# stella-cv/stella_vslam

Measured on AMD Instinct MI355X. Metric: frames/s ORB-extract+match @640x480,2k kpts, higher is better.
Workload: dtype u8

## Files before the change

stella_vslam_amd/csrc/orb_kernels.hip:

```cpp
#include "svgpu_internal.h"
#include "sv_trig.h"
#include <utility>

#pragma clang fp contract(off)

namespace {

__device__ __constant__ float c_pattern_f[1024] = {
#include "orb_pattern_i8.inc"
};

__device__ __forceinline__ int find_level(const OrbLevel* __restrict__ L, int num_levels, int idx, int OrbLevel::*first,
                                          int* local) {
    int lv = 0;
    for (int l = 0; l < num_levels; ++l) {
        const int f = L[l].*first;
        if (idx >= f) lv = l;
    }
    *local = idx - L[lv].*first;
    return lv;
}

__device__ __forceinline__ int reflect101(int p, int len) {
    if (len == 1) return 0;
// ... 261 lines not shown
    }
    else if (MODE == BLUR_EDGE) {
        if (e.left) {
            const uint32_t* p = reinterpret_cast<const uint32_t*>(row);
            r.w1 = p[0];
            r.w2 = p[1];
            r.w0 = __builtin_amdgcn_perm(r.w2, r.w1, 0x01020304u);
        }
        else {
            const uint32_t* p = reinterpret_cast<const uint32_t*>(row + x0 - 4);
            const uint32_t pm1 = p[0], p0 = p[1], p1 = e.hi_p1 ? p[2] : 0u;
            r.w0 = pm1;
            r.w1 = __builtin_amdgcn_perm(p0, pm1, e.sel1);
            r.w2 = e.hi_p1 ? __builtin_amdgcn_perm(p1, p0, e.sel2) : __builtin_amdgcn_perm(p0, pm1, e.sel2);
        }
    }
    else {
        uint32_t b[12];
#pragma unroll
        for (int k = 0; k < 12; ++k) b[k] = row[reflect101(x0 - 4 + k, w)];
        r.w0 = b[0] | (b[1] << 8) | (b[2] << 16) | (b[3] << 24);
        r.w1 = b[4] | (b[5] << 8) | (b[6] << 16) | (b[7] << 24);
        r.w2 = b[8] | (b[9] << 8) | (b[10] << 16) | (b[11] << 24);
    }
    return r;
}
constexpr uint32_t BLUR_TAPS[7] = {18, 34, 48, 56, 48, 34, 18};
constexpr uint32_t blur_tap_word(int j, int word) {
    uint32_t t = 0;
    for (int k = 0; k < 4; ++k) {
        const int i = 4 * word + k - j - 1;
        if (i >= 0 && i < 7) t |= BLUR_TAPS[i] << (8 * k);
    }
    return t;
}
static_assert(blur_tap_word(0, 0) == 0x30221200u && blur_tap_word(0, 1) == 0x12223038u && blur_tap_word(0, 2) == 0u && blur_tap_word(3, 0) == 0u &&
              blur_tap_word(3, 1) == 0x38302212u && blur_tap_word(3, 2) == 0x00122230u, "blur tap words");
template <int J>
__device__ __forceinline__ uint32_t blur_hsum(const BlurRow& r) {
    constexpr uint32_t t0 = blur_tap_word(J, 0), t1 = blur_tap_word(J, 1), t2 = blur_tap_word(J, 2);
    uint32_t s = __builtin_amdgcn_udot4(r.w1, t1, 0u, false);
    if (t0) s = __builtin_amdgcn_udot4(r.w0, t0, s, false);
    if (t2) s = __builtin_amdgcn_udot4(r.w2, t2, s, false);
    return s;
}
__device__ __forceinline__ void blur_hpair(const BlurRow& a, const BlurRow& b, u16x2 (&hp)[4]) {
    hp[0] = as_u16x2(blur_hsum<0>(a) | (blur_hsum<0>(b) << 16));
    hp[1] = as_u16x2(blur_hsum<1>(a) | (blur_hsum<1>(b) << 16));
    hp[2] = as_u16x2(blur_hsum<2>(a) | (blur_hsum<2>(b) << 16));
    hp[3] = as_u16x2(blur_hsum<3>(a) | (blur_hsum<3>(b) << 16));
}
__device__ __forceinline__ uint32_t blur_dot(u16x2 h, uint32_t taps, uint32_t acc) { return __builtin_amdgcn_udot2(h, as_u16x2(taps), acc, false); }
__device__ __forceinline__ uint32_t blur_pack(const uint32_t (&acc)[4]) {
    const uint32_t lo = __builtin_amdgcn_perm(acc[1], acc[0], 0x0c0c0602u), hi = __builtin_amdgcn_perm(acc[3], acc[2], 0x06020c0cu);
    return lo | hi;
}

template <int MODE, int PAIRS = 0, class LoadPair>
__device__ __forceinline__ void blur_walk(LoadPair load_pair, uint8_t* __restrict__ Dp, int dpitch, int ys, int ye) {
    constexpr int AHEAD = MODE == BLUR_LDS ? 0 : 2;
    u16x2 A[4], B[4], C[4], D[4], E[4];
    BlurRow n0 = {}, n1 = {};
    {
        BlurRow r[8];
#pragma unroll
        for (int k = 0; k < 4; ++k) load_pair(ys - 4 + 2 * k, r[2 * k], r[2 * k + 1]);
        if (AHEAD) load_pair(ys + 4, n0, n1);
        if (MODE == BLUR_INTERIOR) {
#pragma unroll
            for (int k = 0; k < 8; ++k) asm volatile("" : "+v"(r[k].w0), "+v"(r[k].w1), "+v"(r[k].w2));
            asm volatile("" : "+v"(n0.w0), "+v"(n0.w1), "+v"(n0.w2), "+v"(n1.w0), "+v"(n1.w1), "+v"(n1.w2));
        }
        blur_hpair(r[0], r[1], A);
        blur_hpair(r[2], r[3], B);
        blur_hpair(r[4], r[5], C);
        blur_hpair(r[6], r[7], D);
    }
    auto step = [&](int y, bool second) {
        const BlurRow c0 = n0, c1 = n1;
        load_pair(y + 4 + AHEAD, n0, n1);
        if (AHEAD) blur_hpair(c0, c1, E);
        else blur_hpair(n0, n1, E);
        uint32_t acc[4];
#pragma unroll
        for (int j = 0; j < 4; ++j)
            acc[j] = blur_dot(D[j], 34u | (18u << 16), blur_dot(C[j], 56u | (48u << 16), blur_dot(B[j], 34u | (48u << 16), blur_dot(A[j], 18u << 16, 32768u))));
        *reinterpret_cast<uint32_t*>(Dp + __umul24(y, dpitch)) = blur_pack(acc);
        if (second) {
#pragma unroll
            for (int j = 0; j < 4; ++j)
                acc[j] = blur_dot(E[j], 18u, blur_dot(D[j], 48u | (34u << 16), blur_dot(C[j], 48u | (56u << 16), blur_dot(B[j], 18u | (34u << 16), 32768u))));
            *reinterpret_cast<uint32_t*>(Dp + __umul24(y + 1, dpitch)) = blur_pack(acc);
        }
#pragma unroll
        for (int j = 0; j < 4; ++j) {
            A[j] = B[j];
            B[j] = C[j];
            C[j] = D[j];
            D[j] = E[j];
        }
    };
    if constexpr (PAIRS > 0) {
#pragma unroll
        for (int i = 0; i < PAIRS; ++i) step(ys + 2 * i, true);
    }
    else
        for (int y = ys; y < ye; y += 2) step(y, y + 1 < ye);
}
template <int MODE>
__device__ __forceinline__ void blur_strip(const uint8_t* __restrict__ src, int spitch, int w, int h, uint8_t* __restrict__ dst,
                                           int dpitch, int x0, int ys, int ye) {
    auto row_ptr = [&](int y) { return src + __umul24(reflect101(y, h), spitch); };
    BlurEdge edge = {};
    if (MODE == BLUR_EDGE) edge = blur_edge_ctx(x0, w);
    blur_walk<MODE>([&](int y, BlurRow& a, BlurRow& b) {
        a = blur_load<MODE>(row_ptr(y), x0, w, edge);
        b = blur_load<MODE>(row_ptr(y + 1), x0, w, edge);
    }, dst + x0, dpitch, ys, ye);
}

__device__ __forceinline__ void blur_locate(const OrbLevel* __restrict__ L, int num_levels, const uint8_t* __restrict__ img0,
                                            size_t img0_frame_stride, int img0_pitch, const uint8_t* __restrict__ pyr,
                                            size_t pyr_frame_bytes, uint8_t* __restrict__ blur, size_t blur_frame_bytes, OrbLevel& lev,
                                            int& tile, const uint8_t*& src, int& spitch, uint8_t*& dst,
                                            int OrbLevel::*first = &OrbLevel::btile_first) {
    int b, item;
    xcd_frame_map(gridDim.x, gridDim.y, item, b);
    const int lv = find_level(L, num_levels, item, first, &tile);
    lev = L[lv];
    if (lv == 0) {
        src = img0 + (size_t)b * img0_frame_stride;
        spitch = img0_pitch;
    }
    else {
        src = pyr + (size_t)b * pyr_frame_bytes + lev.pyr_off;
        spitch = lev.pitch;
    }
    dst = blur + (size_t)b * blur_frame_bytes + lev.blur_off;
}
__device__ __forceinline__ bool blur_streamable(const uint8_t* src, int spitch, int w) {
    return ((((size_t)src) | (size_t)spitch) & 3) == 0 && w >= 16;
}
template <int ROWS>
__global__ __launch_bounds__(256) void k_blur(const OrbLevel* __restrict__ L, int num_levels, const uint8_t* __restrict__ img0,
                                              size_t img0_frame_stride, int img0_pitch, const uint8_t* __restrict__ pyr,
                                              size_t pyr_frame_bytes, uint8_t* __restrict__ blur, size_t blur_frame_bytes) {
    OrbLevel lev;
    int tile, spitch;
    const uint8_t* src;
    uint8_t* dst;
    blur_locate(L, num_levels, img0, img0_frame_stride, img0_pitch, pyr, pyr_frame_bytes, blur, blur_frame_bytes, lev, tile, src, spitch, dst);
    if (!blur_streamable(src, spitch, lev.w)) return;
    const int main_tiles = lev.btiles_x * lev.btiles_y;
    if (tile < main_tiles) {
        const int tx = tile % lev.btiles_x, ty = tile / lev.btiles_x;
        const int rem_groups = tx == lev.btiles_x - 1 ? (min(lev.w - 6, (tx + 1) * BLUR_TW) - tx * BLUR_TW + 3) / 4 : 64;
        int g = 64;
        while (g > 1 && (g >> 1) >= rem_groups) g >>= 1;
        if (g <= 32 && rem_groups > 0) {
            const int spw = 64 / g, lane = threadIdx.x & 63;
            if (ty * spw >= lev.btiles_y) return;
            const int strip = (ty * 4 + (int)(threadIdx.x >> 6)) * spw + lane / g;
            const int x0 = tx * BLUR_TW + (lane % g) * 4, ys = strip * ROWS;
            if (x0 >= lev.w || ys >= lev.h) return;
            if (x0 >= 4 && x0 + 6 < lev.w) blur_strip<BLUR_INTERIOR>(src, spitch, lev.w, lev.h, dst, lev.pitch, x0, ys, min(ys + ROWS, lev.h));
            return;
        }
        const int x0 = tx * BLUR_TW + (threadIdx.x & 63) * 4;
        const int ys = __builtin_amdgcn_readfirstlane(ty * (4 * ROWS) + (int)(threadIdx.x >> 6) * ROWS);
        if (x0 >= lev.w || ys >= lev.h) return;
        if (x0 >= 4 && x0 + 6 < lev.w) blur_strip<BLUR_INTERIOR>(src, spitch, lev.w, lev.h, dst, lev.pitch, x0, ys, min(ys + ROWS, lev.h));
    }
    else {
        const int which = threadIdx.x & 3, strip = (tile - main_tiles) * 64 + (threadIdx.x >> 2);
        const int ys = strip * BLUR_EDGE_ROWS;
        const int last = ((lev.w - 1) >> 2) << 2;
        int x0;
        if (which == 0) x0 = 0;
        else if (which == 1) x0 = last;
        else if (which == 2) x0 = last - 4;
        else return;
        if (ys >= lev.h || x0 < 0 || (which != 0 && (x0 == 0 || x0 + 6 < lev.w))) return;
        blur_strip<BLUR_EDGE>(src, spitch, lev.w, lev.h, dst, lev.pitch, x0, ys, min(ys + BLUR_EDGE_ROWS, lev.h));
    }
}
#define BLUR_LP (16 + BLUR_SEG + 16)
#define BLUR_LDS_ROWS (BLUR_ROWS + 8)
static_assert(BLUR_SEG % 16 == 0 && BLUR_BAND_THREADS % 64 == 0 && BLUR_SEG / 4 <= BLUR_BAND_THREADS && BLUR_ROWS % 2 == 0, "blur band geometry");
static_assert(BLUR_LDS_ROWS * BLUR_LP <= 64 * 1024, "blur band exceeds the static LDS limit");
constexpr int blur_chunks(int groups, int rows) {
    const int fit = BLUR_BAND_THREADS / groups, pairs = rows >> 1, c = fit < pairs ? fit : pairs;
    return c > 1 ? c : 1;
}
constexpr int blur_chunk_rows(int groups, int rows) { return ((rows + blur_chunks(groups, rows) - 1) / blur_chunks(groups, rows) + 1) & ~1; }
constexpr int BLUR_FULL_RC = blur_chunk_rows(BLUR_SEG / 4, BLUR_ROWS);
template <>
__global__ __launch_bounds__(BLUR_BAND_THREADS) void k_blur<BLUR_ROWS>(const OrbLevel* __restrict__ L, int num_levels, const uint8_t* __restrict__ img0,
                                                                       size_t img0_frame_stride, int img0_pitch, const uint8_t* __restrict__ pyr,
                                                                       size_t pyr_frame_bytes, uint8_t* __restrict__ blur, size_t blur_frame_bytes) {
    __shared__ __attribute__((aligned(16))) uint8_t s_rows[BLUR_LDS_ROWS * BLUR_LP];
    OrbLevel lev;
    int item, spitch;
    const uint8_t* src;
    uint8_t* dst;
    blur_locate(L, num_levels, img0, img0_frame_stride, img0_pitch, pyr, pyr_frame_bytes, blur, blur_frame_bytes, lev, item, src, spitch, dst,
                &OrbLevel::bband_first);
    if (!blur_streamable(src, spitch, lev.w)) return;
    const int tid = threadIdx.x, w = lev.w, h = lev.h;
    const int seg = item % lev.bband_segs, xs = seg * BLUR_SEG, sw = min(BLUR_SEG, w - xs);
    const int y0 = (item / lev.bband_segs) * BLUR_ROWS, rows = min(BLUR_ROWS, h - y0);
    const int groups = (sw + 3) >> 2, xend = xs + 4 * groups + 4;
    {
        constexpr int CPR = BLUR_LP / 16;
        const int total = (rows + 6) * CPR;
        const unsigned long long base = (unsigned long long)(uintptr_t)src;
        const uint32_t lds0 = __builtin_amdgcn_readfirstlane((uint32_t)(uintptr_t)(const __attribute__((address_space(3))) uint8_t*)s_rows) + BLUR_LP;
        for (int q0 = __builtin_amdgcn_readfirstlane(tid & ~63); q0 < total; q0 += BLUR_BAND_THREADS) {
            const int q = q0 + (tid & 63), k = q / CPR, x = xs - 16 + 16 * (q - k * CPR);
            if (q < total && x >= 0 && x < min(w, xend)) {
                const uint32_t off = __umul24(reflect101(y0 - 3 + k, h), spitch) + (uint32_t)x;
                if (x + 16 <= w) sv_glds16(base, off, lds0 + 16u * (uint32_t)q0);
                else
#pragma clang loop vectorize(disable)
                    for (int d = 0; x + 4 * d < w; ++d)
                        *reinterpret_cast<uint32_t*>(s_rows + BLUR_LP + 16 * q + 4 * d) = *reinterpret_cast<const uint32_t*>(src + off + 4 * d);
            }
        }
        asm volatile("s_waitcnt vmcnt(0)" ::: "memory");
    }
    __syncthreads();
    for (int i = tid; i < (rows + 6) * 8; i += BLUR_BAND_THREADS) {
        uint8_t* row = s_rows + ((i >> 3) + 1) * BLUR_LP + 16 - xs;
        const int j = i & 7;
        if (j == 0 && xs == 0) {
            const uint32_t* p = reinterpret_cast<const uint32_t*>(row);
            reinterpret_cast<uint32_t*>(row)[-1] = __builtin_amdgcn_perm(p[1], p[0], 0x01020304u);
        }
        const int x = w - 1 + j;
        if (j > 0 && x < xend) row[x] = row[2 * (w - 1) - x];
    }
    __syncthreads();
    const int chunks = blur_chunks(groups, rows), rc = blur_chunk_rows(groups, rows);
    const int c = (int)(((float)tid + 0.5f) * (1.0f / (float)groups)), g = tid - __mul24(c, groups);
    const int r0 = __mul24(c, rc), r1 = min(r0 + rc, rows);
    if (r0 >= r1) return;
    const uint32_t* S = reinterpret_cast<const uint32_t*>(s_rows + 12 + 4 * g);
    auto load_pair = [&](int y, BlurRow& a, BlurRow& b) {
        const uint32_t* p = S + __mul24(y + 4, BLUR_LP / 4);
        a = BlurRow{p[0], p[1], p[2]};
        b = BlurRow{p[BLUR_LP / 4], p[BLUR_LP / 4 + 1], p[BLUR_LP / 4 + 2]};
    };
    uint8_t* const Dp = dst + __umul24(y0, lev.pitch) + xs + 4 * g;
    if (rc == BLUR_FULL_RC && chunks * rc == rows) blur_walk<BLUR_LDS, BLUR_FULL_RC / 2>(load_pair, Dp, lev.pitch, r0, r1);
    else blur_walk<BLUR_LDS>(load_pair, Dp, lev.pitch, r0, r1);
}
template <int ROWS>
__global__ __launch_bounds__(256) void k_blur_gather(const OrbLevel* __restrict__ L, int num_levels, const uint8_t* __restrict__ img0,
                                                     size_t img0_frame_stride, int img0_pitch, const uint8_t* __restrict__ pyr,
                                                     size_t pyr_frame_bytes, uint8_t* __restrict__ blur, size_t blur_frame_bytes) {
    OrbLevel lev;
    int tile, spitch;
    const uint8_t* src;
    uint8_t* dst;
    blur_locate(L, num_levels, img0, img0_frame_stride, img0_pitch, pyr, pyr_frame_bytes, blur, blur_frame_bytes, lev, tile, src, spitch, dst);
    if (blur_streamable(src, spitch, lev.w) || tile >= lev.btiles_x * lev.btiles_y) return;
    const int x0 = (tile % lev.btiles_x) * BLUR_TW + (threadIdx.x & 63) * 4;
    const int ys = (tile / lev.btiles_x) * (4 * ROWS) + (threadIdx.x >> 6) * ROWS;
    if (x0 >= lev.w || ys >= lev.h) return;
    blur_strip<BLUR_GATHER>(src, spitch, lev.w, lev.h, dst, lev.pitch, x0, ys, min(ys + ROWS, lev.h));
}

typedef short s16x2 __attribute__((ext_vector_type(2)));
__device__ __forceinline__ int arc_score16(int v, const int (&p)[16]) {
    s16x2 e[16];
#pragma unroll
    for (int k = 0; k < 16; ++k) e[k] = __builtin_bit_cast(s16x2, __mul24(p[k], -65535) + (int)0xFFFF0000);
    s16x2 m2[8], m4[8];
#pragma unroll
    for (int j = 0; j < 8; ++j) m2[j] = __builtin_elementwise_min(e[2 * j + 1], e[(2 * j + 2) & 15]);
#pragma unroll
    for (int j = 0; j < 8; ++j) m4[j] = __builtin_elementwise_min(m2[j], m2[(j + 1) & 7]);
    s16x2 best = s16x2{(short)-32768, (short)-32768};
#pragma unroll
    for (int j = 0; j < 8; ++j) {
        const s16x2 m8 = __builtin_elementwise_min(m4[j], m4[(j + 2) & 7]);
        best = __builtin_elementwise_max(best, __builtin_elementwise_min(m8, __builtin_elementwise_max(e[2 * j], e[(2 * j + 9) & 15])));
    }
    return max(max((int)best.x - v, v + 1 + (int)best.y), 0);
}

#define FAST_KT 12
#define FP 80
__global__ __launch_bounds__(256) void k_fast(const OrbLevel* __restrict__ L, int num_levels, const FastCell* __restrict__ cells, int num_cells, int cpw,
                                              const uint8_t* __restrict__ img0, size_t img0_frame_stride, int img0_pitch,
                                              const uint8_t* __restrict__ pyr, size_t pyr_frame_bytes,
                                              const unsigned short* __restrict__ gtab, unsigned long long* __restrict__ keys,
                                              int total_grid, int ini_thr, int min_thr, const uint8_t* __restrict__ mask,
                                              size_t mask_frame_stride, int mask_pitch, int mask_w, int mask_h) {
    __shared__ __attribute__((aligned(16))) uint8_t s_raw[SV_ROI_MAX * FP + 16];
    __shared__ __attribute__((aligned(16))) uint8_t s_a[SV_ROI_MAX * FP];
    __shared__ unsigned short s_q[SV_CELL * SV_CELL];
    __shared__ unsigned long long s_key[FAST_KT * FAST_KT];
    __shared__ unsigned short s_gx[SV_ROI_MAX], s_gy[SV_ROI_MAX];
    __shared__ int s_count;
    int b, grp;
    xcd_frame_map(gridDim.x, gridDim.y, grp, b);
    const int tid = threadIdx.x, lane = tid & 63;
    const int wv = __builtin_amdgcn_readfirstlane(tid >> 6);
    const uint8_t* M = mask ? mask + (size_t)b * mask_frame_stride : nullptr;
    const uint8_t* const I0 = img0 + (size_t)b * img0_frame_stride;
    const uint8_t* const PY = pyr + (size_t)b * pyr_frame_bytes;
    unsigned long long* const KF = keys + (size_t)b * total_grid;
    uint8_t* const s_img = s_raw + 3;
    unsigned short* const my_q = s_q + wv * (SV_CELL * SV_CELL / 4);
    const int qrow = lane >> 4, qk = lane & 15;
    const int x0 = 3 + 4 * qk;
    const int ly0 = 3 + 4 * (4 * qrow + wv);
    const int e0 = (ly0 << 7) | x0;
    const uint32_t* const qbase = reinterpret_cast<const uint32_t*>(s_raw + ly0 * FP + 4 * qk);

    auto load_ring = [&](const uint8_t* c, int (&p)[16]) {
        p[0] = c[3 * FP];
        p[1] = c[3 * FP + 1];
        p[2] = c[2 * FP + 2];
        p[3] = c[FP + 3];
        p[4] = c[3];
        p[5] = c[-FP + 3];
        p[6] = c[-2 * FP + 2];
        p[7] = c[-3 * FP + 1];
        p[8] = c[-3 * FP];
        p[9] = c[-3 * FP - 1];
        p[10] = c[-2 * FP - 2];
        p[11] = c[-FP - 3];
        p[12] = c[-3];
        p[13] = c[FP - 3];
        p[14] = c[2 * FP - 2];
        p[15] = c[3 * FP - 1];
    };

    const int c_first = grp * cpw, c_last = min(c_first + cpw, num_cells);
    for (int ci = c_first; ci < c_last; ++ci) {
    const FastCell cell = cells[ci];
    const OrbLevel lev = L[cell.lv];
    auto masked = [&](int y, int x) -> bool {
        int my = (int)((float)y * lev.scale), mx = (int)((float)x * lev.scale);
        my = min(my, mask_h - 1);
        mx = min(mx, mask_w - 1);
        return M[(size_t)my * mask_pitch + mx] == 0;
    };
    if (M) {
        const int y0 = cell.min_y, y1 = cell.min_y + cell.h, xa = cell.min_x, xb = cell.min_x + cell.w;
        if (masked(y0, xa) || masked(y1, xa) || masked(y0, xb) || masked(y1, xb)) continue;
    }
    const uint8_t* src;
    int spitch;
    if (cell.lv == 0) {
        src = I0;
        spitch = img0_pitch;
    }
    else {
        src = PY + lev.pyr_off;
        spitch = lev.pitch;
    }
    const int w = cell.w, h = cell.h;
    if (ci != c_first) __syncthreads();
    const uint8_t* rsrc = src + (size_t)cell.min_y * spitch + (cell.min_x - 3);
    {
        const unsigned long long rbase = (unsigned long long)(uintptr_t)rsrc;
        const uint32_t lds_raw = __builtin_amdgcn_readfirstlane((uint32_t)(uintptr_t)(const __attribute__((address_space(3))) uint8_t*)s_raw) + (uint32_t)wv * 1024u;
#pragma unroll
        for (int it = 0; it < 2; ++it) {
            const int q = tid + 256 * it, r = q / 5, c = q - 5 * r;
            if (it == 0 || wv < 2) {
                if (q < SV_ROI_MAX * (FP / 16) && r < h && 16 * c < w + 3) sv_glds16(rbase, (uint32_t)(__umul24(r, spitch) + 16 * c), lds_raw + 4096u * it);
            }
            if (q < SV_ROI_MAX * (FP / 16)) reinterpret_cast<uint4*>(s_a)[q] = make_uint4(0, 0, 0, 0);
        }
    }
    if (tid == 0) {
        s_count = 0;
    }
    if (tid < FAST_KT * FAST_KT) s_key[tid] = 0ull;
    if (tid < w) s_gx[tid] = gtab[lev.gtab_x_off + cell.min_x + tid - SV_PATCH_RADIUS];
    else if (tid >= 128 && tid - 128 < h) s_gy[tid - 128] = gtab[lev.gtab_y_off + cell.min_y + (tid - 128) - SV_PATCH_RADIUS];
    uint32_t band80 = 0;
#pragma unroll
    for (int j = 0; j < 4; ++j) band80 |= (x0 + j < w - 3) ? (0x80u << (8 * j)) : 0u;
    asm volatile("s_waitcnt vmcnt(0)" ::: "memory");
    __syncthreads();

    unsigned long long* K = KF + lev.grid_first;
    const int gx0 = s_gx[3], gy0 = s_gy[3];
    for (int pass = 0; pass < 2; ++pass) {
    const int t = pass == 0 ? ini_thr : min_thr, tq = t;
    int wq = 0;
#if defined(FAST_ABLATE) && FAST_ABLATE >= 2
    if (mask_h == -12345)
#endif
    {
        const uint32_t tqq = (uint32_t)(tq + 1) * 0x10001u;
        uint32_t m = 0;
#pragma unroll
        for (int g = 0; g < 4; ++g) {
            const uint32_t* const rc = qbase + g * (FP / 4);
            const uint32_t w0 = rc[0], w1 = rc[1], w2 = rc[2], w3 = rc[3];
            const uint32_t d1 = rc[3 * (FP / 4) + 1], d2 = rc[3 * (FP / 4) + 2], u1 = rc[-3 * (FP / 4) + 1], u2 = rc[-3 * (FP / 4) + 2];
            auto pk = [](uint32_t hi, uint32_t lo, uint32_t sel) { return __builtin_bit_cast(s16x2, __builtin_amdgcn_perm(hi, lo, sel)); };
            uint32_t e2[2];
#pragma unroll
            for (int half = 0; half < 2; ++half) {
                const s16x2 v = pk(w2, w1, half ? 0x0c050c04u : 0x0c030c02u);
                const s16x2 p0 = pk(d2, d1, half ? 0x0c050c04u : 0x0c030c02u);
                const s16x2 p8 = pk(u2, u1, half ? 0x0c050c04u : 0x0c030c02u);
                const s16x2 p12 = pk(w1, w0, half ? 0x0c060c05u : 0x0c040c03u);
                const s16x2 p4 = pk(w3, w2, half ? 0x0c040c03u : 0x0c020c01u);
                const s16x2 up = __builtin_elementwise_min(__builtin_elementwise_max(p0, p8), __builtin_elementwise_max(p4, p12));
                const s16x2 dn = __builtin_elementwise_max(__builtin_elementwise_min(p0, p8), __builtin_elementwise_min(p4, p12));
                const s16x2 mm = __builtin_elementwise_max(up - v, v - dn);
                e2[half] = __builtin_bit_cast(uint32_t, mm - __builtin_bit_cast(s16x2, tqq));
            }
            const uint32_t sgn = __builtin_amdgcn_perm(e2[1], e2[0], 0x07050301u);
            m = (m >> 1) | (~sgn & (ly0 + g < h - 3 ? band80 : 0u));
        }
        const int cnt = __popc(m);
        int incl = cnt;
        incl += __builtin_amdgcn_update_dpp(0, incl, 0x111, 0xF, 0xF, false);
        incl += __builtin_amdgcn_update_dpp(0, incl, 0x112, 0xF, 0xF, false);
        incl += __builtin_amdgcn_update_dpp(0, incl, 0x114, 0xF, 0xF, false);
        incl += __builtin_amdgcn_update_dpp(0, incl, 0x118, 0xF, 0xF, false);
        incl += __builtin_amdgcn_update_dpp(0, incl, 0x142, 0xA, 0xF, false);
        incl += __builtin_amdgcn_update_dpp(0, incl, 0x143, 0xC, 0xF, false);
        wq = __builtin_amdgcn_readlane(incl, 63);
        int pos = incl - cnt;
        while (m) {
            const int bit = __ffs((int)m) - 1;
            m &= m - 1;
            my_q[pos++] = (unsigned short)(e0 + (((bit & 7) - 4) << 7) + (bit >> 3));
        }
    }
#if defined(FAST_ABLATE) && FAST_ABLATE >= 1
    if (mask_h != -12345) wq = 0;
#endif
    __builtin_amdgcn_fence(__ATOMIC_RELEASE, "wavefront");
    __builtin_amdgcn_wave_barrier();
    __builtin_amdgcn_fence(__ATOMIC_ACQUIRE, "wavefront");
    for (int i = lane; i < wq; i += 64) {
        const int e = my_q[i], ly = e >> 7, qx = e & 127;
        const uint8_t* c = &s_img[ly * FP + qx];
        int p[16];
        load_ring(c, p);
        s_a[ly * FP + qx] = (uint8_t)arc_score16(c[0], p);
    }
    __syncthreads();

    {
        int found = 0;
        for (int i = lane; i < wq; i += 64) {
            const int e = my_q[i], ly = e >> 7, qx = e & 127;
            const uint8_t* a = &s_a[ly * FP + qx];
            const int A = a[0];
            if (A <= t) continue;
            const int s = A - 1;
            const int n0 = max(max((int)a[-FP - 1], (int)a[-FP]), (int)a[-FP + 1]);
            const int n1 = max(max((int)a[-1], (int)a[1]), (int)a[FP - 1]);
            const int n2 = max(max((int)a[FP], (int)a[FP + 1]), n0);
            const bool keep = A > 1 && max(n1, n2) < A;
            if (!keep) continue;
            ++found;
            const int x_level = cell.min_x + qx, y_level = cell.min_y + ly;
            if (M && masked(y_level, x_level)) continue;
            const int gx = s_gx[qx], gy = s_gy[ly];
            const uint32_t order = (uint32_t)cell.order_base | ((uint32_t)ly << 7) | (uint32_t)qx;
            const unsigned long long key = ((unsigned long long)(uint32_t)s << 32) | (0xFFFFFFFFu - order);
            const int kx = gx - gx0, ky = gy - gy0;
            if ((unsigned)kx < FAST_KT && (unsigned)ky < FAST_KT) atomicMax(&s_key[ky * FAST_KT + kx], key);
            else atomicMax(&K[gy * lev.grid_x + gx], key);
        }
        if (found) atomicAdd(&s_count, found);
        __syncthreads();
        if (s_count > 0) break;
        __syncthreads();
    }
    }
    if (tid < FAST_KT * FAST_KT) {
        const unsigned long long key = s_key[tid];
        if (key) atomicMax(&K[(gy0 + tid / FAST_KT) * lev.grid_x + gx0 + tid % FAST_KT], key);
    }
    }
}

__global__ __launch_bounds__(1024) void k_select(const OrbLevel* __restrict__ L, int num_levels, unsigned long long* __restrict__ keys,
                                                 int total_grid, int4* __restrict__ sel, int32_t* __restrict__ counts, int32_t* __restrict__ cellpos) {
    __shared__ int s_wave[16], s_lvcnt[SV_MAX_LEVELS];
    const int b = blockIdx.x, tid = threadIdx.x, lane = tid & 63, wave = tid >> 6;
    unsigned long long* K = keys + (size_t)b * total_grid;
    int4* S = sel + (size_t)b * total_grid;
    if (tid < SV_MAX_LEVELS) s_lvcnt[tid] = 0;
    int running = 0;
    for (int base = 0; base < total_grid; base += 1024) {
        const int idx = base + tid;
        unsigned long long key = 0;
        if (idx < total_grid) {
            key = K[idx];
            if (key) K[idx] = 0;
        }
        const unsigned long long bal = __ballot(key != 0);
        const int before = __popcll(bal & ((1ull << lane) - 1ull));
        __syncthreads();
        if (lane == 0) s_wave[wave] = __popcll(bal);
        __syncthreads();
        int woff = 0, total = 0;
#pragma unroll
        for (int k = 0; k < 16; ++k) {
            if (k < wave) woff += s_wave[k];
            total += s_wave[k];
        }
        if (cellpos && idx < total_grid) cellpos[(size_t)b * (total_grid + 1) + idx] = running + woff + before;
        if (key) {
            int lv = 0;
            while (lv + 1 < num_levels && idx >= L[lv + 1].grid_first) ++lv;
            const uint32_t order = 0xFFFFFFFFu - (uint32_t)(key & 0xFFFFFFFFu);
            const int lx = order & 127, ly = (order >> 7) & 127, cid = order >> 14;
            const int cells_x = L[lv].cells_x;
            const int ci = cid / cells_x, cj = cid - ci * cells_x;
            int4 r;
            r.x = SV_PATCH_RADIUS + cj * SV_CELL + lx;
            r.y = SV_PATCH_RADIUS + ci * SV_CELL + ly;
            r.z = lv;
            r.w = (int)(key >> 32);
            S[running + woff + before] = r;
            atomicAdd(&s_lvcnt[lv], 1);
        }
        running += total;
    }
    __syncthreads();
    if (tid < num_levels) counts[b * (1 + num_levels) + 1 + tid] = s_lvcnt[tid];
    if (tid == 0) {
        counts[b * (1 + num_levels)] = running;
        if (cellpos) cellpos[(size_t)b * (total_grid + 1) + total_grid] = running;
    }
}

__device__ __forceinline__ float dev_fast_atan2(float y, float x) {
    const float p1 = 0.9997878412794807f * (float)(180 / 3.1415926535897932384626433832795);
    const float p3 = -0.3258083974640975f * (float)(180 / 3.1415926535897932384626433832795);
    const float p5 = 0.1555786518463281f * (float)(180 / 3.1415926535897932384626433832795);
    const float p7 = -0.04432655554792128f * (float)(180 / 3.1415926535897932384626433832795);
    const float eps = (float)2.2204460492503131e-16;
    const float ax = fabsf(x), ay = fabsf(y);
    float a, c, c2;
    if (ax >= ay) {
        c = ay / (ax + eps);
        c2 = c * c;
        a = (((p7 * c2 + p5) * c2 + p3) * c2 + p1) * c;
    }
    else {
        c = ax / (ay + eps);
        c2 = c * c;
        a = 90.f - (((p7 * c2 + p5) * c2 + p3) * c2 + p1) * c;
    }
    if (x < 0) a = 180.f - a;
    if (y < 0) a = 360.f - a;
    return a;
}

__device__ __forceinline__ float dev_util_cos(float v) { return sv_util_cos(v); }
__device__ __forceinline__ float dev_util_sin(float v) { return sv_util_sin(v); }

__device__ __forceinline__ int wave_sum(int v) {
    v += __builtin_amdgcn_update_dpp(0, v, 0x111, 0xF, 0xF, false);
    v += __builtin_amdgcn_update_dpp(0, v, 0x112, 0xF, 0xF, false);
    v += __builtin_amdgcn_update_dpp(0, v, 0x114, 0xF, 0xF, false);
    v += __builtin_amdgcn_update_dpp(0, v, 0x118, 0xF, 0xF, false);
    v += __builtin_amdgcn_update_dpp(0, v, 0x142, 0xA, 0xF, false);
    v += __builtin_amdgcn_update_dpp(0, v, 0x143, 0xC, 0xF, false);
    return __builtin_amdgcn_readlane(v, 63);
}

#ifndef DESC_KPW
#define DESC_KPW 5
#endif
#define DESC_IP 32
#define DESC_BP 40
#define DESC_R 18
#define DESC_SLAB (DESC_KPW * 37 * DESC_BP + 16)
struct IcWeights {
    uint32_t w1[256], wu[256];
};
constexpr IcWeights make_ic_weights() {
    constexpr int umax[16] = {15, 15, 15, 15, 14, 14, 14, 13, 13, 12, 11, 10, 9, 8, 6, 3};
    IcWeights t{};
    for (int row = 0; row < 31; ++row)
        for (int j = 0; j < 8; ++j) {
            uint32_t w1 = 0, wu = 0;
            const int v = row - 15, av = v < 0 ? -v : v;
            for (int k = 0; k < 4; ++k) {
                const int col = 4 * j + k, u = col - 15, au = u < 0 ? -u : u;
                if (col < 31 && au <= umax[av]) {
                    w1 |= 1u << (8 * k);
                    wu |= (uint32_t)(u + 15) << (8 * k);
                }
            }
            t.w1[row * 8 + j] = w1;
            t.wu[row * 8 + j] = wu;
        }
    return t;
}
__device__ __constant__ IcWeights c_icw = make_ic_weights();

__global__ __launch_bounds__(256) void k_describe(const OrbLevel* __restrict__ L, int num_levels, const int4* __restrict__ sel,
                                                  int total_grid, const int32_t* __restrict__ counts,
                                                  const uint8_t* __restrict__ img0, size_t img0_frame_stride, int img0_pitch,
                                                  const uint8_t* __restrict__ pyr, size_t pyr_frame_bytes,
                                                  const uint8_t* __restrict__ blur, size_t blur_frame_bytes,
                                                  svgpu_keypoint* __restrict__ kps, uint8_t* __restrict__ desc, int cap, float* __restrict__ angles) {
    __shared__ __attribute__((aligned(16))) uint8_t s_slab[4][DESC_SLAB];
    int b, blk;
    xcd_frame_map(gridDim.x, gridDim.y, blk, b);
    const int lane = threadIdx.x & 63, wave = __builtin_amdgcn_readfirstlane(threadIdx.x >> 6);
    const int n = min(counts[b * (1 + num_levels)], cap);
    const int i0 = (blk * 4 + wave) * DESC_KPW;
    if (i0 >= n) return;
    uint8_t* const slab = s_slab[wave];
    float px0[4], py0[4], px1[4], py1[4];
#pragma unroll
    for (int r = 0; r < 4; ++r) {
        const float4 q = reinterpret_cast<const float4*>(c_pattern_f)[r * 64 + lane];
        px0[r] = q.x;
        py0[r] = q.y;
        px1[r] = q.z;
        py1[r] = q.w;
    }
    uint32_t w1[4], wu[4];
    int rowv[4];
#pragma unroll
    for (int m = 0; m < 4; ++m) {
        const int item = lane + 64 * m;
        w1[m] = c_icw.w1[item];
        wu[m] = c_icw.wu[item];
        rowv[m] = (item >> 3) - 15;
    }
    const int nk = min(DESC_KPW, n - i0);
    const int4* const S = sel + (size_t)b * total_grid + i0;
    const uint8_t* const I0 = img0 + (size_t)b * img0_frame_stride;
    const uint8_t* const PY = pyr + (size_t)b * pyr_frame_bytes;
    const uint8_t* const BL = blur + (size_t)b * blur_frame_bytes;
    const int part = lane & 3, prow = lane >> 2;
    const int br = lane / 5, bpart = lane - 5 * br;
    int4 sv[DESC_KPW];
#pragma unroll
    for (int kk = 0; kk < DESC_KPW; ++kk) sv[kk] = S[kk];
    const uint8_t* gi[DESC_KPW];
    const uint8_t* gbl[DESC_KPW];
    int pit_i[DESC_KPW], pit_b[DESC_KPW];
#pragma unroll
    for (int kk = 0; kk < DESC_KPW; ++kk) {
        const int lv = kk < nk ? sv[kk].z : 0;
        pit_b[kk] = L[lv].pitch;
        pit_i[kk] = lv == 0 ? img0_pitch : pit_b[kk];
        gi[kk] = (lv == 0 ? I0 : PY + L[lv].pyr_off) + (size_t)(sv[kk].y - 15) * pit_i[kk] + (sv[kk].x - 15);
        gbl[kk] = BL + L[lv].blur_off + (size_t)(sv[kk].y - DESC_R) * pit_b[kk] + (sv[kk].x - DESC_R);
    }
    uint2 vi[DESC_KPW][2];
#pragma unroll
    for (int kk = 0; kk < DESC_KPW; ++kk)
        if (kk < nk) {
#pragma unroll
            for (int h = 0; h < 2; ++h)
                if (16 * h + prow < 31) __builtin_memcpy(&vi[kk][h], gi[kk] + (__umul24(16 * h + prow, pit_i[kk]) + 8 * part), 8);
        }
#pragma unroll
    for (int kk = 0; kk < DESC_KPW; ++kk)
        if (kk < nk) {
#pragma unroll
            for (int h = 0; h < 2; ++h)
                if (16 * h + prow < 31) *reinterpret_cast<uint2*>(slab + kk * (31 * DESC_IP) + (16 * h + prow) * DESC_IP + 8 * part) = vi[kk][h];
        }
    __builtin_amdgcn_fence(__ATOMIC_RELEASE, "wavefront");
    __builtin_amdgcn_wave_barrier();
    __builtin_amdgcn_fence(__ATOMIC_ACQUIRE, "wavefront");
    uint2 vb[DESC_KPW][4];
#pragma unroll
    for (int kk = 0; kk < DESC_KPW; ++kk)
        if (kk < nk) {
#pragma unroll
            for (int h = 0; h < 4; ++h)
                if (br < 12 && 12 * h + br < 37) __builtin_memcpy(&vb[kk][h], gbl[kk] + (__umul24(12 * h + br, pit_b[kk]) + 8 * bpart), 8);
        }
    int my10 = 0, my01 = 0;
#pragma unroll
    for (int kk = 0; kk < DESC_KPW; ++kk)
        if (kk < nk) {
            int m10 = 0, m01 = 0;
#pragma unroll
            for (int m = 0; m < 4; ++m) {
                const int item = lane + 64 * m;
                const uint32_t px = item < 248 ? reinterpret_cast<const uint32_t*>(slab + kk * (31 * DESC_IP))[item] : 0u;
                const int s1 = (int)__builtin_amdgcn_udot4(px, w1[m], 0u, false), su = (int)__builtin_amdgcn_udot4(px, wu[m], 0u, false);
                m10 += su - __mul24(15, s1);
                m01 += __mul24(rowv[m], s1);
            }
            m10 = wave_sum(m10);
            m01 = wave_sum(m01);
            if (lane == kk) {
                my10 = m10;
                my01 = m01;
            }
        }
    const float angle = dev_fast_atan2((float)my01, (float)my10);
    const float rad = (float)((double)angle * 3.14159265358979323846 / 180.0);
    const float ca_l = dev_util_cos(rad), sa_l = dev_util_sin(rad);
    __builtin_amdgcn_fence(__ATOMIC_RELEASE, "wavefront");
    __builtin_amdgcn_wave_barrier();
#pragma unroll
    for (int kk = 0; kk < DESC_KPW; ++kk)
        if (kk < nk) {
#pragma unroll
            for (int h = 0; h < 4; ++h)
                if (br < 12 && 12 * h + br < 37) *reinterpret_cast<uint2*>(slab + kk * (37 * DESC_BP) + __mul24(12 * h + br, DESC_BP) + 8 * bpart) = vb[kk][h];
        }
    __builtin_amdgcn_fence(__ATOMIC_RELEASE, "wavefront");
    __builtin_amdgcn_wave_barrier();
    __builtin_amdgcn_fence(__ATOMIC_ACQUIRE, "wavefront");
#pragma unroll
    for (int kk = 0; kk < DESC_KPW; ++kk)
        if (kk < nk) {
            const float ca = __int_as_float(__builtin_amdgcn_readlane(__float_as_int(ca_l), kk));
            const float sa = __int_as_float(__builtin_amdgcn_readlane(__float_as_int(sa_l), kk));
            const uint8_t* B = slab + kk * (37 * DESC_BP) + DESC_R * DESC_BP + DESC_R;
            unsigned long long bits[4];
#pragma unroll
            for (int r = 0; r < 4; ++r) {
                const float x0 = px0[r], y0 = py0[r], x1 = px1[r], y1 = py1[r];
                constexpr float RN = 12582912.0f;
                constexpr int RK = 0x400000 * DESC_BP + 0x4B400000;
                typedef float f32x2 __attribute__((ext_vector_type(2)));
                const f32x2 sc = {sa, ca}, cs = {ca, -sa}, rn = {RN, RN};
                const f32x2 q0 = (f32x2{x0, x0} * sc + f32x2{y0, y0} * cs) + rn;
                const f32x2 q1 = (f32x2{x1, x1} * sc + f32x2{y1, y1} * cs) + rn;
                const int r0 = __float_as_int(q0.x), c0 = __float_as_int(q0.y);
                const int r1 = __float_as_int(q1.x), c1 = __float_as_int(q1.y);
                const int a = B[__mul24(r0, DESC_BP) + c0 - RK];
                const int bb = B[__mul24(r1, DESC_BP) + c1 - RK];
                bits[r] = __builtin_amdgcn_ballot_w64(a < bb);
            }
            uint8_t* D = desc + ((size_t)b * cap + i0 + kk) * 32;
            if (lane < 4) reinterpret_cast<unsigned long long*>(D)[lane] = lane == 0 ? bits[0] : lane == 1 ? bits[1] : lane == 2 ? bits[2] : bits[3];
        }
    if (lane < nk) {
        const int4 s = S[lane];
        const int lv = s.z;
        svgpu_keypoint k;
        k.x = (float)s.x;
        k.y = (float)s.y;
        if (lv != 0) {
            k.x = k.x * L[lv].scale;
            k.y = k.y * L[lv].scale;
        }
        k.size = L[lv].kp_size;
        k.angle = angle;
        k.response = (float)s.w;
        k.octave = lv;
        k.class_id = -1;
        kps[(size_t)b * cap + i0 + lane] = k;
// ... 262 lines not shown
```

Measured before the change: 283,400.

## Balance FAST candidate scoring across waves and compact corners before NMS

Replaces the per-wave scoring loop with a block-wide loop over all four waves' candidate queues, using prefix sums of per-wave counts to map global indices into the queue slots. This spreads uneven candidate counts across waves. Candidates that pass the threshold are compacted in place with ballot/mbcnt, so the NMS pass only visits real corners, also spread across the whole block. It adds a block barrier and slot-mapping arithmetic, and the in-place compaction relies on write indices never overtaking read indices.

```diff
diff --git a/stella_vslam_amd/csrc/orb_kernels.hip b/stella_vslam_amd/csrc/orb_kernels.hip
--- a/stella_vslam_amd/csrc/orb_kernels.hip
+++ b/stella_vslam_amd/csrc/orb_kernels.hip
@@ -587,7 +587,7 @@
     __shared__ unsigned short s_q[SV_CELL * SV_CELL];
     __shared__ unsigned long long s_key[FAST_KT * FAST_KT];
     __shared__ unsigned short s_gx[SV_ROI_MAX], s_gy[SV_ROI_MAX];
-    __shared__ int s_count;
+    __shared__ int s_count, s_wq[4], s_wc[4];
     int b, grp;
     xcd_frame_map(gridDim.x, gridDim.y, grp, b);
     const int tid = threadIdx.x, lane = tid & 63;
@@ -726,25 +726,47 @@
 #if defined(FAST_ABLATE) && FAST_ABLATE >= 1
     if (mask_h != -12345) wq = 0;
 #endif
-    __builtin_amdgcn_fence(__ATOMIC_RELEASE, "wavefront");
-    __builtin_amdgcn_wave_barrier();
-    __builtin_amdgcn_fence(__ATOMIC_ACQUIRE, "wavefront");
-    for (int i = lane; i < wq; i += 64) {
-        const int e = my_q[i], ly = e >> 7, qx = e & 127;
-        const uint8_t* c = &s_img[ly * FP + qx];
-        int p[16];
-        load_ring(c, p);
-        s_a[ly * FP + qx] = (uint8_t)arc_score16(c[0], p);
-    }
+    if (lane == 0) s_wq[wv] = wq;
+    __syncthreads();
+    const int QW = SV_CELL * SV_CELL / 4;
+    const int P1 = __builtin_amdgcn_readfirstlane(s_wq[0]), P2 = P1 + __builtin_amdgcn_readfirstlane(s_wq[1]),
+              P3 = P2 + __builtin_amdgcn_readfirstlane(s_wq[2]), total = P3 + __builtin_amdgcn_readfirstlane(s_wq[3]);
+    const int o1 = QW - P1, o2 = 2 * QW - P2, o3 = 3 * QW - P3;
+    auto slot = [=](int v) { return v + (v < P2 ? (v < P1 ? 0 : o1) : (v < P3 ? o2 : o3)); };
+    int cw = 0;
+    for (int i0 = wv * 64; i0 < total; i0 += 256) {
+        const int i = i0 + lane;
+        int e = 0;
+        bool corner = false;
+        if (i < total) {
+            e = s_q[slot(i)];
+            const int ly = e >> 7, qx = e & 127;
+            const uint8_t* c = &s_img[ly * FP + qx];
+            int p[16];
+            load_ring(c, p);
+            const int A = arc_score16(c[0], p);
+            s_a[ly * FP + qx] = (uint8_t)A;
+            corner = A > t;
+        }
+        const unsigned long long hit = __ballot(corner);
+        if (corner) {
+            const int j = cw + (int)__builtin_amdgcn_mbcnt_hi((uint32_t)(hit >> 32), __builtin_amdgcn_mbcnt_lo((uint32_t)hit, 0u));
+            s_q[slot(((j >> 6) << 8) + (wv << 6) + (j & 63))] = (unsigned short)e;
+        }
+        cw += __popcll(hit);
+    }
+    if (lane == 0) s_wc[wv] = cw;
     __syncthreads();
 
     {
         int found = 0;
-        for (int i = lane; i < wq; i += 64) {
-            const int e = my_q[i], ly = e >> 7, qx = e & 127;
+        const int C1 = __builtin_amdgcn_readfirstlane(s_wc[0]), C2 = C1 + __builtin_amdgcn_readfirstlane(s_wc[1]),
+                  C3 = C2 + __builtin_amdgcn_readfirstlane(s_wc[2]), ctotal = C3 + __builtin_amdgcn_readfirstlane(s_wc[3]);
+        for (int i = tid; i < ctotal; i += 256) {
+            const int j = i - (i < C1 ? 0 : i < C2 ? C1 : i < C3 ? C2 : C3), cwv64 = i < C1 ? 0 : i < C2 ? 64 : i < C3 ? 128 : 192;
+            const int e = s_q[slot(((j >> 6) << 8) + cwv64 + (j & 63))], ly = e >> 7, qx = e & 127;
             const uint8_t* a = &s_a[ly * FP + qx];
             const int A = a[0];
-            if (A <= t) continue;
             const int s = A - 1;
             const int n0 = max(max((int)a[-FP - 1], (int)a[-FP]), (int)a[-FP + 1]);
             const int n1 = max(max((int)a[-1], (int)a[1]), (int)a[FP - 1]);
```

Result: slower. 278,600 (-1.7%).
